# jizongFox/MI-based-Regularized-Semi-supervised-Segmentation

Hardware: NVIDIA B200
Metric: iic_mi_loss_fwd_bwd_mpixels_per_s (higher is better)
Workload: dtype f32

## Files before the change

### mi-based-regularized-semi-supervised-segmentation_b200/csrc/local_bwd_tcrb10h.cu

```cuda
#include <cuda_fp16.h>
#include <stdlib.h>

#include "common.cuh"
#include "local_kernels.cuh"
#include "tc_common.cuh"
#include "tma.cuh"

namespace iic {
namespace bwdrb10h {
using namespace tc;

constexpr int T = 3, PAD = 1;
constexpr int KP = 16;
constexpr int RMAX = 8;
constexpr int TBUF = 2 * RMAX * KP;
constexpr int APX = 272;
constexpr int MAXW = 248;
constexpr int A_CHUNK = APX * 16;
constexpr int A_SLOT = 4 * A_CHUNK;
constexpr int NA = 6;
constexpr int RAW_SLOT = 10 * 256 * 4;
constexpr int NRAW = 6;
constexpr int WROWS = T * KP;
constexpr int W_TILE = 2 * WROWS * 16;
constexpr int W_IMG = 6 * W_TILE;
constexpr int NTHREADS = 704;
constexpr int NTHREADS_FL = 704;
constexpr int SMEM_BYTES = NA * A_SLOT + 2 * W_IMG + NRAW * RAW_SLOT + 1024;
constexpr int NL = 4;
constexpr int SMEM_BYTES_FL = SMEM_BYTES + NL * RAW_SLOT;
constexpr float A_SCALE = 256.f;
constexpr int A_SCALE_LOG2 = 8;
constexpr int W_TARGET_LOG2 = 12;



#ifdef IIC_TC_TRACE
__device__ long long g_trace[4][64][6];
__device__ long long g_ctrace[32][8];
#define TRACE(role, slot) do { if (blockIdx.x == 0 && tt >= 16 && tt < 80) g_trace[role][tt - 16][slot] = clock64(); } while (0)
#define CTRACE(slot) do { if (blockIdx.x == 0 && i < 32) g_ctrace[i][slot] = clock64(); } while (0)
#else
#define TRACE(role, slot) do { } while (0)
#define CTRACE(slot) do { } while (0)
#endif

struct Params {
  int B, H, W, K;
  const float* Wc[2];
  int Kp4;
  const float* grad_loss;
  float* out[2];
  long long out_sn[2];
  int from_logits;
  float inv_temp;
  const float* lout[2];
  long long l_sn[2], l_sc[2], l_sh[2];
};

__device__ __forceinline__ uint32_t pack_h2(float a, float b) {
  const __half2 p = __floats2half2_rn(a, b);
  return *reinterpret_cast<const uint32_t*>(&p);
}
__device__ __forceinline__ uint4 pack_h8(const float* v) {
  return make_uint4(pack_h2(v[0], v[1]), pack_h2(v[2], v[3]), pack_h2(v[4], v[5]), pack_h2(v[6], v[7]));
}
__device__ __forceinline__ void split_h(float v, float& h, float& l) {
  h = __half2float(__float2half_rn(v));
  l = __half2float(__float2half_rn(v - h));
}

__device__ __forceinline__ void build_weight_row(const float* __restrict__ Wc, unsigned char* img, int e, int K, int Kp4, float wscale) {
  const int row = e % WROWS, tx = e / WROWS;
  const int ty = T - 1 - row / KP, o = row % KP;
  float w1[10], w2[10];
#pragma unroll
  for (int c = 0; c < 10; ++c) {
    const float v = (c < K && o < K) ? __ldg(Wc + ((size_t)c * T * T + ty * T + tx) * Kp4 + o) * wscale : 0.f;
    split_h(v, w1[c], w2[c]);
  }
  const float c0[8] = {w1[0], w1[1], w1[2], w1[3], w1[4], w1[5], w1[6], w1[7]};
  const float c1[8] = {w1[8], w1[9], w1[0], w1[1], w1[2], w1[3], w1[4], w1[5]};
  const float c2[8] = {w1[6], w1[7], w1[8], w1[9], w2[0], w2[1], w2[2], w2[3]};
  const float c3[8] = {w2[4], w2[5], w2[6], w2[7], w2[8], w2[9], 0.f, 0.f};
  uint4* t = reinterpret_cast<uint4*>(img + (size_t)tx * 2 * W_TILE);
  t[row] = pack_h8(c0);
  t[WROWS + row] = pack_h8(c1);
  t[2 * WROWS + row] = pack_h8(c2);
  t[3 * WROWS + row] = pack_h8(c3);
}

struct Chunk { int n, h0, nr, q0; bool cont_next; };
__device__ __forceinline__ Chunk next_chunk(long long r, long long R0, long long R1, int H, int rc) {
  Chunk c;
  c.n = (int)(r / H);
  c.h0 = (int)(r - (long long)c.n * H);
  int run = H - c.h0;
  if (run > R1 - r) run = (int)(R1 - r);
  c.nr = rc < run ? rc : run;
  if (run - c.nr == 1 && c.nr >= 3) c.nr -= 1;
  c.q0 = (r > R0 && c.h0 > 0) ? 2 : 0;
  c.cont_next = c.nr < run;
  return c;
}

template <bool FROM_LOGITS>
__global__ void __launch_bounds__(FROM_LOGITS ? NTHREADS_FL : NTHREADS, 1)
local_bwd_tcrb10h_kernel(const __grid_constant__ CUtensorMap map0, const __grid_constant__ CUtensorMap map1, const Params P) {
  extern __shared__ __align__(1024) unsigned char smem_dyn[];
  __shared__ __align__(8) uint64_t raw_full[NRAW], raw_empty[NRAW], a_full[NA], a_empty[NA], w_full, accum_full[2], tmem_ready[2];
  __shared__ __align__(8) uint64_t l_full[NL], l_empty[NL];
  __shared__ uint32_t tmem_base_s;
  __shared__ float wmax_s[4];
  __shared__ float unscale_s;
  unsigned char* smem = smem_dyn + ((1024u - (smem_u32(smem_dyn) & 1023u)) & 1023u);
  unsigned char* a_ring = smem;
  unsigned char* w_img = smem + NA * A_SLOT;
  unsigned char* raw_ring = w_img + 2 * W_IMG;
  unsigned char* l_ring = raw_ring + NRAW * RAW_SLOT;
  const int wid = threadIdx.x >> 5, lane = threadIdx.x & 31;
  const long long rows_total = (long long)P.B * P.H;
  const long long R0 = (long long)blockIdx.x * rows_total / gridDim.x;
  const long long R1 = (long long)(blockIdx.x + 1) * rows_total / gridDim.x;
  const int share = (int)(R1 - R0);
  const int nch = (share + RMAX - 1) / RMAX;
  const int rc = nch > 0 ? (share + nch - 1) / nch : RMAX;
  const int SW = P.W + 8;
  const int raw_bytes = P.K * SW * 4;
  const int ntile = P.W > 128 ? 2 : 1;

  if (threadIdx.x == 0) {
    for (int s = 0; s < NRAW; ++s) { mbar_init(&raw_full[s], 1); mbar_init(&raw_empty[s], 4); }
    for (int s = 0; s < NA; ++s) { mbar_init(&a_full[s], 4); mbar_init(&a_empty[s], 2); }
    mbar_init(&w_full, 4);
    const int ndset_i = ntile == 2 ? 2 : 1;
    for (int s = 0; s < 2; ++s) { mbar_init(&accum_full[s], 4); mbar_init(&tmem_ready[s], 4 * ndset_i); }
    for (int s = 0; s < NL; ++s) { mbar_init(&l_full[s], 1); mbar_init(&l_empty[s], 4 * ndset_i); }
    mbar_fence_init();
  }
  if (wid == 3) {
    asm volatile("tcgen05.alloc.cta_group::1.sync.aligned.shared::cta.b32 [%0], %1;" ::"r"(smem_u32(&tmem_base_s)), "r"(512));
    asm volatile("tcgen05.relinquish_alloc_permit.cta_group::1.sync.aligned;");
  }
  asm volatile("tcgen05.fence::before_thread_sync;");
  __syncthreads();
  asm volatile("tcgen05.fence::after_thread_sync;");
  const uint32_t tmem_base = tmem_base_s;

  if (wid == 0) {
    if (lane == 0) {
      tma_prefetch_desc(&map0);
      tma_prefetch_desc(&map1);
      int t = 0, s = 0;
      unsigned sph = 0;
      for (int sweep = 0; sweep < 2; ++sweep)
      for (long long r = R0; r < R1;) {
        const Chunk c = next_chunk(r, R0, R1, P.H, rc);
        for (int q = c.q0; q < c.nr + T - 1; ++q, ++t) {
          { const int tt = t; (void)tt; TRACE(0, 0); }
          if (t >= NRAW) mbar_wait(&raw_empty[s], sph ^ 1u, 1);
          { const int tt = t; (void)tt; TRACE(0, 1); }
          mbar_arrive_expect_tx(&raw_full[s], raw_bytes);
          tma_load_4d(raw_ring + s * RAW_SLOT, sweep == 0 ? &map0 : &map1, &raw_full[s], -4, c.h0 - PAD + q, 0, c.n);
          if (++s == NRAW) { s = 0; sph ^= 1u; }
        }
        r += c.nr;
      }
    }
  } else if (wid == 3) {
    if (FROM_LOGITS && lane == 0) {
      int t = 0, s = 0;
      unsigned sph = 0;
      for (int sweep = 0; sweep < 2; ++sweep)
      for (long long r = R0; r < R1;) {
        const Chunk c = next_chunk(r, R0, R1, P.H, rc);
        for (int orow = 0; orow < c.nr; ++orow, ++t) {
          if (t >= NL) mbar_wait(&l_empty[s], sph ^ 1u, 9);
          mbar_arrive_expect_tx(&l_full[s], raw_bytes);
          tma_load_4d(l_ring + s * RAW_SLOT, sweep == 0 ? &map1 : &map0, &l_full[s], -4, c.h0 + orow, 0, c.n);
          if (++s == NL) { s = 0; sph ^= 1u; }
        }
        r += c.nr;
      }
    }
  } else if (wid == 1 || wid == 2 || wid == 12 || wid == 13) {
    const int mt = (wid == 1 || wid == 12) ? 0 : 1;
    const int par = wid >= 12 ? 1 : 0;
    const bool mine = mt < ntile;
    mbar_wait(&w_full, 0u, 7);
    const uint64_t w_base0 = make_desc_kmajor_noswz(smem_u32(w_img), WROWS * 16);
    static_assert(NA % 2 == 0 && NRAW % 2 == 0, "the stage-parity split needs even ring depths");
    int a = 0, i = 0, tt = 0;
    unsigned aph = 0;
    for (int sweep = 0; sweep < 2; ++sweep)
    for (long long r = R0; r < R1; ++i) {
      const uint64_t w_base = w_base0 + (uint64_t)(sweep * (W_IMG / 16));
      const Chunk c = next_chunk(r, R0, R1, P.H, rc);
      const int buf = i & 1;
      if (lane == 0 && wid == 1) CTRACE(0);
      mbar_wait(&tmem_ready[buf], (unsigned)(i >> 1) & 1u, 6);
      if (lane == 0 && wid == 1) CTRACE(1);
      asm volatile("tcgen05.fence::after_thread_sync;");
      const int nq = c.nr + T - 1;
      const int nr_next = c.cont_next ? next_chunk(r + c.nr, R0, R1, P.H, rc).nr : 0;
      for (int q = c.q0; q < nq; ++q, ++tt) {
        if ((tt & 1) != par) {
          if (++a == NA) { a = 0; aph ^= 1u; }
          continue;
        }
        if (lane == 0 && par == 0) TRACE(1 + mt, 0);
        mbar_wait(&a_full[a], aph, 5);
        asm volatile("tcgen05.fence::after_thread_sync;");
        if (lane == 0) {
          if (par == 0) TRACE(1 + mt, 1);
          if (mine) {
            const int ty_max = q < T - 1 ? q : T - 1;
            const int ty_min = q - c.nr + 1 > 0 ? q - c.nr + 1 : 0;
            const uint32_t nn = (uint32_t)((ty_max - ty_min + 1) * KP);
            const uint32_t idesc_f16 = (1u << 4) | ((nn >> 3) << 17) | (8u << 24);
            const uint32_t d_tmem = tmem_base + (uint32_t)(buf * TBUF + (mt * RMAX + (q - ty_max)) * KP);
            const uint64_t a_12 = make_desc_kmajor_noswz(smem_u32(a_ring + a * A_SLOT), A_CHUNK) + (uint64_t)(mt * 128 + 8 - PAD);
            const uint64_t a_34 = a_12 + (uint64_t)(2 * A_CHUNK / 16);
            const uint64_t b_base = w_base + (uint64_t)((T - 1 - ty_max) * KP);
#pragma unroll
            for (int tx = 0; tx < T; ++tx) {
              const uint64_t bt = b_base + (uint64_t)tx * (2 * W_TILE / 16);
              umma_bf16(d_tmem, a_12 + (uint64_t)tx, bt, idesc_f16);
              umma_bf16(d_tmem, a_34 + (uint64_t)tx, bt + (uint64_t)(W_TILE / 16), idesc_f16);
            }
          }
        }
        if (c.cont_next && q >= c.nr) {
          mbar_wait(&tmem_ready[buf ^ 1], (unsigned)((i + 1) >> 1) & 1u, 6);
          asm volatile("tcgen05.fence::after_thread_sync;");
          if (lane == 0 && mine) {
            const int q2 = q - c.nr;
            const int ty_max = q2;
            const int ty_min = q2 - nr_next + 1 > 0 ? q2 - nr_next + 1 : 0;
            const uint32_t nn = (uint32_t)((ty_max - ty_min + 1) * KP);
            const uint32_t idesc_f16 = (1u << 4) | ((nn >> 3) << 17) | (8u << 24);
            const uint32_t d_tmem = tmem_base + (uint32_t)((buf ^ 1) * TBUF + (mt * RMAX + (q2 - ty_max)) * KP);
            const uint64_t a_12 = make_desc_kmajor_noswz(smem_u32(a_ring + a * A_SLOT), A_CHUNK) + (uint64_t)(mt * 128 + 8 - PAD);
            const uint64_t a_34 = a_12 + (uint64_t)(2 * A_CHUNK / 16);
            const uint64_t b_base = w_base + (uint64_t)((T - 1 - ty_max) * KP);
#pragma unroll
            for (int tx = 0; tx < T; ++tx) {
              const uint64_t bt = b_base + (uint64_t)tx * (2 * W_TILE / 16);
              umma_bf16(d_tmem, a_12 + (uint64_t)tx, bt, idesc_f16);
              umma_bf16(d_tmem, a_34 + (uint64_t)tx, bt + (uint64_t)(W_TILE / 16), idesc_f16);
            }
          }
        }
        if (lane == 0) {
          if (par == 0) TRACE(1 + mt, 2);
          umma_commit(&a_empty[a]);
        }
        __syncwarp();
        if (++a == NA) { a = 0; aph ^= 1u; }
      }
      if (lane == 0) umma_commit(&accum_full[buf]);
      __syncwarp();
      r += c.nr;
    }
  } else if (wid >= 4 && wid < 12) {
    const int tid = (threadIdx.x - 128) & 127;
    const int grp = wid >= 8 ? 1 : 0;
    int a = 0, s = 0, t = 0;
    unsigned aph = 0, sph = 0;
    for (int sweep = 0; sweep < 2; ++sweep)
    for (long long r = R0; r < R1;) {
      const Chunk c = next_chunk(r, R0, R1, P.H, rc);
      for (int q = c.q0; q < c.nr + T - 1; ++q, ++t) {
        if ((t & 1) != grp) {
          if (++a == NA) { a = 0; aph ^= 1u; }
          if (++s == NRAW) { s = 0; sph ^= 1u; }
          continue;
        }
        const int tt = t;
        (void)tt;
        if (tid == 0 && wid == 4) TRACE(3, 0);
        if (t >= NA) mbar_wait(&a_empty[a], aph ^ 1u, 3);
        if (tid == 0 && wid == 4) TRACE(3, 1);
        mbar_wait(&raw_full[s], sph, 4);
        if (tid == 0 && wid == 4) TRACE(3, 2);
        unsigned char* am = a_ring + a * A_SLOT;
        const float* raw = reinterpret_cast<const float*>(raw_ring + s * RAW_SLOT);
        const int srow = c.h0 - PAD + q;
        const bool row_in = srow >= 0 && srow < P.H;
        float v[2][10];
#pragma unroll
        for (int u = 0; u < 2; ++u) {
          const int px = tid + u * 128;
#pragma unroll
          for (int ch = 0; ch < 10; ++ch) v[u][ch] = (ch < P.K && px < SW) ? raw[ch * SW + px] : 0.f;
        }
#pragma unroll
        for (int u = 0; u < 2; ++u) {
          const int px = tid + u * 128;
          if (FROM_LOGITS) {
            const int col = px - 4;
            if (row_in && col >= 0 && col < P.W) {
              float mx = v[u][0];
#pragma unroll
              for (int ch = 1; ch < 10; ++ch) if (ch < P.K) mx = fmaxf(mx, v[u][ch]);
              float sum = 0.f;
#pragma unroll
              for (int ch = 0; ch < 10; ++ch) {
                v[u][ch] = ch < P.K ? __expf((v[u][ch] - mx) * P.inv_temp) : 0.f;
                sum += v[u][ch];
              }
              const float inv = 1.f / sum;
#pragma unroll
              for (int ch = 0; ch < 10; ++ch) v[u][ch] *= inv;
            } else {
#pragma unroll
              for (int ch = 0; ch < 10; ++ch) v[u][ch] = 0.f;
            }
          }
        }
        float2 hi[10], lo[10];
#pragma unroll
        for (int ch = 0; ch < 10; ++ch) {
          const float2 sv = __fmul2_rn(make_float2(v[0][ch], v[1][ch]), make_float2(A_SCALE, A_SCALE));
          hi[ch] = make_float2(__uint_as_float(__float_as_uint(sv.x) & 0xFFFFE000u), __uint_as_float(__float_as_uint(sv.y) & 0xFFFFE000u));
          lo[ch] = __ffma2_rn(hi[ch], make_float2(-1.f, -1.f), sv);
        }
#pragma unroll
        for (int u = 0; u < 2; ++u) {
          const int px = tid + u * 128;
          uint32_t hp[5], lp[5];
#pragma unroll
          for (int c2 = 0; c2 < 5; ++c2) {
            const __half2 hh = u == 0 ? __floats2half2_rn(hi[2 * c2].x, hi[2 * c2 + 1].x) : __floats2half2_rn(hi[2 * c2].y, hi[2 * c2 + 1].y);
            const __half2 ll = u == 0 ? __floats2half2_rn(lo[2 * c2].x, lo[2 * c2 + 1].x) : __floats2half2_rn(lo[2 * c2].y, lo[2 * c2 + 1].y);
            hp[c2] = *reinterpret_cast<const uint32_t*>(&hh);
            lp[c2] = *reinterpret_cast<const uint32_t*>(&ll);
          }
          if (px < SW) {
            const int off = (px + 4) * 16;
            *reinterpret_cast<uint4*>(am + off) = make_uint4(hp[0], hp[1], hp[2], hp[3]);
            *reinterpret_cast<uint4*>(am + A_CHUNK + off) = make_uint4(hp[4], lp[0], lp[1], lp[2]);
            *reinterpret_cast<uint4*>(am + 2 * A_CHUNK + off) = make_uint4(lp[3], lp[4], hp[0], hp[1]);
            *reinterpret_cast<uint4*>(am + 3 * A_CHUNK + off) = make_uint4(hp[2], hp[3], hp[4], 0u);
          }
        }
        __syncwarp();
        if (lane == 0) mbar_arrive(&raw_empty[s]);
        asm volatile("fence.proxy.async.shared::cta;" ::: "memory");
        __syncwarp();
        if (lane == 0) mbar_arrive(&a_full[a]);
        if (tid == 0 && wid == 4) TRACE(3, 3);
        if (++a == NA) { a = 0; aph ^= 1u; }
        if (++s == NRAW) { s = 0; sph ^= 1u; }
      }
      r += c.nr;
    }
  } else if (wid >= 14) {
    const int q4 = wid & 3;
    const int dset = wid >= 18 ? 1 : 0;
    const int ndset = ntile == 2 ? 2 : 1;
    const int mt0 = ndset == 2 ? dset : 0, mt1 = ndset == 2 ? dset + 1 : ntile;
    const int zc0 = ndset == 2 ? dset * RMAX * KP : 0, zc1 = ndset == 2 ? (dset + 1) * RMAX * KP : TBUF;
    float unscale = 1.f;
    const float g0 = P.grad_loss ? __ldg(P.grad_loss) : 1.f;
    const size_t plane = (size_t)P.H * P.W;
    const uint32_t lane_base = tmem_base + ((uint32_t)(q4 * 32) << 16);
    auto zero_accumulators = [&](int buf) {
      for (int c = zc0; c < zc1; c += 8)
        asm volatile("tcgen05.st.sync.aligned.32x32b.x8.b32 [%0], {%1, %1, %1, %1, %1, %1, %1, %1};" ::"r"(lane_base + buf * TBUF + c), "r"(0u) : "memory");
      asm volatile("tcgen05.wait::st.sync.aligned;" ::: "memory");
      asm volatile("tcgen05.fence::before_thread_sync;");
      __syncwarp();
      if (lane == 0) mbar_arrive(&tmem_ready[buf]);
    };
    if (dset < ndset) {
    zero_accumulators(0);
    zero_accumulators(1);
    }
    if (dset == 0) {
      const int etid = threadIdx.x - 14 * 32;
      const int ncoef = P.K * T * T * P.Kp4;
      float mx = 0.f;
      for (int e = etid; e < 2 * ncoef; e += 128) mx = fmaxf(mx, fabsf(__ldg(P.Wc[e >= ncoef] + (e >= ncoef ? e - ncoef : e))));
#pragma unroll
      for (int o = 16; o > 0; o >>= 1) mx = fmaxf(mx, __shfl_xor_sync(0xffffffffu, mx, o));
      if (lane == 0) wmax_s[q4] = mx;
      asm volatile("bar.sync 1, 128;" ::: "memory");
      mx = fmaxf(fmaxf(wmax_s[0], wmax_s[1]), fmaxf(wmax_s[2], wmax_s[3]));
      int wexp = 0;
      if (mx > 0.f && mx < 3.0e38f) wexp = W_TARGET_LOG2 - ilogbf(mx);
      if (wexp > 100) wexp = 100;
      const float wscale = scalbnf(1.f, wexp);
      unscale = scalbnf(1.f, -(wexp + A_SCALE_LOG2));
      for (int e = etid; e < 2 * 3 * WROWS; e += 128) {
        const int sweep = e / (3 * WROWS);
        build_weight_row(P.Wc[sweep], w_img + sweep * W_IMG, e - sweep * 3 * WROWS, P.K, P.Kp4, wscale);
      }
      if (etid == 0) unscale_s = unscale;
      asm volatile("fence.proxy.async.shared::cta;" ::: "memory");
      __syncwarp();
      if (lane == 0) mbar_arrive(&w_full);
    } else {
      mbar_wait(&w_full, 0u, 7);
      unscale = *reinterpret_cast<volatile float*>(&unscale_s);
    }
    const float g = g0 * unscale;
    int i = 0, ls = 0;
    unsigned lph = 0;
    for (int sweep = 0; sweep < 2 && dset < ndset; ++sweep)
    for (long long r = R0; r < R1; ++i) {
      const Chunk c = next_chunk(r, R0, R1, P.H, rc);
      const int buf = i & 1;
      if (lane == 0 && wid == 14) CTRACE(2);
      mbar_wait(&accum_full[buf], (unsigned)(i >> 1) & 1u, 8);
      if (lane == 0 && wid == 14) CTRACE(3);
      asm volatile("tcgen05.fence::after_thread_sync;");
      for (int orow = 0; orow < c.nr; orow += 2) {
        const int nrow = orow + 1 < c.nr ? 2 : 1;
        if (FROM_LOGITS) {
          mbar_wait(&l_full[ls], lph, 10);
          if (nrow == 2) mbar_wait(&l_full[(ls + 1) % NL], (ls + 1 == NL) ? (lph ^ 1u) : lph, 10);
        }
        for (int mt = mt0; mt < mt1; ++mt) {
          const int col = mt * 128 + q4 * 32 + lane;
          const bool live = col < P.W;
          uint32_t v[2][16];
#pragma unroll
          for (int h = 0; h < 2; ++h) {
            const int orh = orow + h < RMAX ? orow + h : orow;
#pragma unroll
            for (int ch = 0; ch < 16; ch += 8) {
              const uint32_t taddr = lane_base + (uint32_t)(buf * TBUF + (mt * RMAX + orh) * KP + ch);
              asm volatile("tcgen05.ld.sync.aligned.32x32b.x8.b32 {%0, %1, %2, %3, %4, %5, %6, %7}, [%8];"
                           : "=r"(v[h][ch]), "=r"(v[h][ch + 1]), "=r"(v[h][ch + 2]), "=r"(v[h][ch + 3]), "=r"(v[h][ch + 4]),
                             "=r"(v[h][ch + 5]), "=r"(v[h][ch + 6]), "=r"(v[h][ch + 7])
                           : "r"(taddr));
            }
          }
          asm volatile("tcgen05.wait::ld.sync.aligned;" ::: "memory");
          if (live) {
#pragma unroll
            for (int h = 0; h < 2; ++h) {
              if (h < nrow) {
                float* dst = P.out[sweep] + (size_t)c.n * P.out_sn[sweep] + (size_t)(c.h0 + orow + h) * P.W + col;
                if (!FROM_LOGITS) {
                  if (P.K == 10) {
#pragma unroll
                    for (int o = 0; o < 10; ++o) dst[(size_t)o * plane] = g * __uint_as_float(v[h][o]);
                  } else {
#pragma unroll
                    for (int o = 0; o < 9; ++o) dst[(size_t)o * plane] = g * __uint_as_float(v[h][o]);
                  }
                } else {
                  const float* lp = reinterpret_cast<const float*>(l_ring + ((ls + h) % NL) * RAW_SLOT) + col + 4;
                  float pr[10];
                  float mx = -3.0e38f;
#pragma unroll
                  for (int o = 0; o < 10; ++o) {
                    pr[o] = o < P.K ? lp[o * SW] : -3.0e38f;
                    mx = fmaxf(mx, pr[o]);
                  }
                  float sum = 0.f;
#pragma unroll
                  for (int o = 0; o < 10; ++o) {
                    pr[o] = o < P.K ? __expf((pr[o] - mx) * P.inv_temp) : 0.f;
                    sum += pr[o];
                  }
                  const float inv = 1.f / sum;
                  float dot = 0.f;
#pragma unroll
                  for (int o = 0; o < 10; ++o) {
                    pr[o] *= inv;
                    dot = fmaf(g * __uint_as_float(v[h][o]), pr[o], dot);
                  }
                  if (P.K == 10) {
#pragma unroll
                    for (int o = 0; o < 10; ++o) dst[(size_t)o * plane] = P.inv_temp * pr[o] * (g * __uint_as_float(v[h][o]) - dot);
                  } else {
#pragma unroll
                    for (int o = 0; o < 9; ++o) dst[(size_t)o * plane] = P.inv_temp * pr[o] * (g * __uint_as_float(v[h][o]) - dot);
                  }
                }
              }
            }
          }
        }
        if (FROM_LOGITS) {
          __syncwarp();
          for (int h = 0; h < nrow; ++h) {
            if (lane == 0) mbar_arrive(&l_empty[ls]);
            if (++ls == NL) { ls = 0; lph ^= 1u; }
          }
        }
      }
      r += c.nr;
      if (lane == 0 && wid == 14) CTRACE(4);
      zero_accumulators(buf);
      if (lane == 0 && wid == 14) CTRACE(5);
    }
  }
  asm volatile("tcgen05.fence::before_thread_sync;");
  __syncthreads();
  if (wid == 3) asm volatile("tcgen05.dealloc.cta_group::1.sync.aligned.b32 %0, %1;" ::"r"(tmem_base), "r"(512));
}

}

int local_bwd_tcrb10h_try(const LocalMaps& m, const float* Wx, const float* Wy, const LocalGrads& g, int from_logits,
                          float inv_temp, cudaStream_t st) {
  using namespace bwdrb10h;
  const int B = m.B, K = m.K, H = m.H, W = m.W, sms = m.sms;
  if ((K != 9 && K != 10) || m.pad != 1 || W % 4 != 0 || W > MAXW || W < 8) return -1;
  if ((long long)B * H < 8LL * sms && !options().tc10_force) return -1;
  CUtensorMap mx, my;
  if (!make_map_4d(&mx, m.x, m, W + 8, 1, K)) return -1;
  if (!make_map_4d(&my, m.y, m, W + 8, 1, K)) return -1;
  IIC_CHECK_RC(ensure_dyn_smem((const void*)(local_bwd_tcrb10h_kernel<false>), (int)(SMEM_BYTES)));
  IIC_CHECK_RC(ensure_dyn_smem((const void*)(local_bwd_tcrb10h_kernel<true>), (int)(SMEM_BYTES_FL)));
  const int Kp4 = (K + 3) & ~3;
  Params P{B, H, W, K, {Wx, Wy}, Kp4, g.grad_loss, {g.gx, g.gy}, {g.gx_sn, g.gy_sn}, from_logits, inv_temp, {m.x.p, m.y.p},
           {m.x.sn, m.y.sn}, {m.x.sc, m.y.sc}, {m.x.sh, m.y.sh}};
  if (from_logits) local_bwd_tcrb10h_kernel<true><<<sms, NTHREADS_FL, SMEM_BYTES_FL, st>>>(my, mx, P);
  else local_bwd_tcrb10h_kernel<false><<<sms, NTHREADS, SMEM_BYTES, st>>>(my, mx, P);
  IIC_CHECK_CUDA(cudaGetLastError());
  return 0;
}

}
```

Before: 10220.

## Fold horizontal conv taps into MMA N dimension and combine shifted outputs in epilogue

Replaces the three per-tx MMAs per row with a single wider MMA whose N dimension packs all three horizontal taps (KP 32, RMAX 4). The epilogue then sums the three tap outputs with lane shuffles, using shared-memory seam exchange across warps, and tiles columns by 126 with halo overlap. The aim is to cut the number of tensor-core instructions and weight-tile traffic per row. In exchange it adds epilogue shuffles, a named barrier per row, halved row depth per accumulator, and an extra A-ring zero-padding pass.

```diff
diff --git a/mi-based-regularized-semi-supervised-segmentation_b200/csrc/local_bwd_tcrb10h.cu b/mi-based-regularized-semi-supervised-segmentation_b200/csrc/local_bwd_tcrb10h.cu
--- a/mi-based-regularized-semi-supervised-segmentation_b200/csrc/local_bwd_tcrb10h.cu
+++ b/mi-based-regularized-semi-supervised-segmentation_b200/csrc/local_bwd_tcrb10h.cu
@@ -11,9 +11,10 @@
 using namespace tc;
 
 constexpr int T = 3, PAD = 1;
-constexpr int KP = 16;
-constexpr int RMAX = 8;
+constexpr int KP = 32;
+constexpr int RMAX = 4;
 constexpr int TBUF = 2 * RMAX * KP;
+constexpr int TILE = 126;
 constexpr int APX = 272;
 constexpr int MAXW = 248;
 constexpr int A_CHUNK = APX * 16;
@@ -23,7 +24,7 @@
 constexpr int NRAW = 6;
 constexpr int WROWS = T * KP;
 constexpr int W_TILE = 2 * WROWS * 16;
-constexpr int W_IMG = 6 * W_TILE;
+constexpr int W_IMG = 2 * W_TILE;
 constexpr int NTHREADS = 704;
 constexpr int NTHREADS_FL = 704;
 constexpr int SMEM_BYTES = NA * A_SLOT + 2 * W_IMG + NRAW * RAW_SLOT + 1024;
@@ -70,20 +71,20 @@
   l = __half2float(__float2half_rn(v - h));
 }
 
-__device__ __forceinline__ void build_weight_row(const float* __restrict__ Wc, unsigned char* img, int e, int K, int Kp4, float wscale) {
-  const int row = e % WROWS, tx = e / WROWS;
-  const int ty = T - 1 - row / KP, o = row % KP;
+__device__ __forceinline__ void build_weight_row(const float* __restrict__ Wc, unsigned char* img, int row, int K, int Kp4, float wscale) {
+  const int ty = T - 1 - row / KP, rr = row % KP;
+  const int tx = rr / 10, o = rr % 10;
   float w1[10], w2[10];
 #pragma unroll
   for (int c = 0; c < 10; ++c) {
-    const float v = (c < K && o < K) ? __ldg(Wc + ((size_t)c * T * T + ty * T + tx) * Kp4 + o) * wscale : 0.f;
+    const float v = (c < K && o < K && tx < T) ? __ldg(Wc + ((size_t)c * T * T + ty * T + tx) * Kp4 + o) * wscale : 0.f;
     split_h(v, w1[c], w2[c]);
   }
   const float c0[8] = {w1[0], w1[1], w1[2], w1[3], w1[4], w1[5], w1[6], w1[7]};
   const float c1[8] = {w1[8], w1[9], w1[0], w1[1], w1[2], w1[3], w1[4], w1[5]};
   const float c2[8] = {w1[6], w1[7], w1[8], w1[9], w2[0], w2[1], w2[2], w2[3]};
   const float c3[8] = {w2[4], w2[5], w2[6], w2[7], w2[8], w2[9], 0.f, 0.f};
-  uint4* t = reinterpret_cast<uint4*>(img + (size_t)tx * 2 * W_TILE);
+  uint4* t = reinterpret_cast<uint4*>(img);
   t[row] = pack_h8(c0);
   t[WROWS + row] = pack_h8(c1);
   t[2 * WROWS + row] = pack_h8(c2);
@@ -113,6 +114,7 @@
   __shared__ uint32_t tmem_base_s;
   __shared__ float wmax_s[4];
   __shared__ float unscale_s;
+  __shared__ float seam_s[2][2][4][2][10];
   unsigned char* smem = smem_dyn + ((1024u - (smem_u32(smem_dyn) & 1023u)) & 1023u);
   unsigned char* a_ring = smem;
   unsigned char* w_img = smem + NA * A_SLOT;
@@ -127,7 +129,7 @@
   const int rc = nch > 0 ? (share + nch - 1) / nch : RMAX;
   const int SW = P.W + 8;
   const int raw_bytes = P.K * SW * 4;
-  const int ntile = P.W > 128 ? 2 : 1;
+  const int ntile = P.W > TILE ? 2 : 1;
 
   if (threadIdx.x == 0) {
     for (int s = 0; s < NRAW; ++s) { mbar_init(&raw_full[s], 1); mbar_init(&raw_empty[s], 4); }
@@ -219,15 +221,11 @@
             const uint32_t nn = (uint32_t)((ty_max - ty_min + 1) * KP);
             const uint32_t idesc_f16 = (1u << 4) | ((nn >> 3) << 17) | (8u << 24);
             const uint32_t d_tmem = tmem_base + (uint32_t)(buf * TBUF + (mt * RMAX + (q - ty_max)) * KP);
-            const uint64_t a_12 = make_desc_kmajor_noswz(smem_u32(a_ring + a * A_SLOT), A_CHUNK) + (uint64_t)(mt * 128 + 8 - PAD);
+            const uint64_t a_12 = make_desc_kmajor_noswz(smem_u32(a_ring + a * A_SLOT), A_CHUNK) + (uint64_t)(mt * TILE + 8 - PAD);
             const uint64_t a_34 = a_12 + (uint64_t)(2 * A_CHUNK / 16);
             const uint64_t b_base = w_base + (uint64_t)((T - 1 - ty_max) * KP);
-#pragma unroll
-            for (int tx = 0; tx < T; ++tx) {
-              const uint64_t bt = b_base + (uint64_t)tx * (2 * W_TILE / 16);
-              umma_bf16(d_tmem, a_12 + (uint64_t)tx, bt, idesc_f16);
-              umma_bf16(d_tmem, a_34 + (uint64_t)tx, bt + (uint64_t)(W_TILE / 16), idesc_f16);
-            }
+            umma_bf16(d_tmem, a_12, b_base, idesc_f16);
+            umma_bf16(d_tmem, a_34, b_base + (uint64_t)(W_TILE / 16), idesc_f16);
           }
         }
         if (c.cont_next && q >= c.nr) {
@@ -240,15 +238,11 @@
             const uint32_t nn = (uint32_t)((ty_max - ty_min + 1) * KP);
             const uint32_t idesc_f16 = (1u << 4) | ((nn >> 3) << 17) | (8u << 24);
             const uint32_t d_tmem = tmem_base + (uint32_t)((buf ^ 1) * TBUF + (mt * RMAX + (q2 - ty_max)) * KP);
-            const uint64_t a_12 = make_desc_kmajor_noswz(smem_u32(a_ring + a * A_SLOT), A_CHUNK) + (uint64_t)(mt * 128 + 8 - PAD);
+            const uint64_t a_12 = make_desc_kmajor_noswz(smem_u32(a_ring + a * A_SLOT), A_CHUNK) + (uint64_t)(mt * TILE + 8 - PAD);
             const uint64_t a_34 = a_12 + (uint64_t)(2 * A_CHUNK / 16);
             const uint64_t b_base = w_base + (uint64_t)((T - 1 - ty_max) * KP);
-#pragma unroll
-            for (int tx = 0; tx < T; ++tx) {
-              const uint64_t bt = b_base + (uint64_t)tx * (2 * W_TILE / 16);
-              umma_bf16(d_tmem, a_12 + (uint64_t)tx, bt, idesc_f16);
-              umma_bf16(d_tmem, a_34 + (uint64_t)tx, bt + (uint64_t)(W_TILE / 16), idesc_f16);
-            }
+            umma_bf16(d_tmem, a_12, b_base, idesc_f16);
+            umma_bf16(d_tmem, a_34, b_base + (uint64_t)(W_TILE / 16), idesc_f16);
           }
         }
         if (lane == 0) {
@@ -265,6 +259,13 @@
   } else if (wid >= 4 && wid < 12) {
     const int tid = (threadIdx.x - 128) & 127;
     const int grp = wid >= 8 ? 1 : 0;
+    {
+      const int npx = APX - (SW + 4);
+      for (int e = tid; e < (NA / 2) * 4 * npx; e += 128) {
+        const int slot = 2 * (e / (4 * npx)) + grp, k = (e / npx) % 4, px = SW + 4 + e % npx;
+        *reinterpret_cast<uint4*>(a_ring + slot * A_SLOT + k * A_CHUNK + px * 16) = make_uint4(0u, 0u, 0u, 0u);
+      }
+    }
     int a = 0, s = 0, t = 0;
     unsigned aph = 0, sph = 0;
     for (int sweep = 0; sweep < 2; ++sweep)
@@ -359,7 +360,7 @@
     const int q4 = wid & 3;
     const int dset = wid >= 18 ? 1 : 0;
     const int ndset = ntile == 2 ? 2 : 1;
-    const int mt0 = ndset == 2 ? dset : 0, mt1 = ndset == 2 ? dset + 1 : ntile;
+    const int mt = dset;
     const int zc0 = ndset == 2 ? dset * RMAX * KP : 0, zc1 = ndset == 2 ? (dset + 1) * RMAX * KP : TBUF;
     float unscale = 1.f;
     const float g0 = P.grad_loss ? __ldg(P.grad_loss) : 1.f;
@@ -392,9 +393,9 @@
       if (wexp > 100) wexp = 100;
       const float wscale = scalbnf(1.f, wexp);
       unscale = scalbnf(1.f, -(wexp + A_SCALE_LOG2));
-      for (int e = etid; e < 2 * 3 * WROWS; e += 128) {
-        const int sweep = e / (3 * WROWS);
-        build_weight_row(P.Wc[sweep], w_img + sweep * W_IMG, e - sweep * 3 * WROWS, P.K, P.Kp4, wscale);
+      for (int e = etid; e < 2 * WROWS; e += 128) {
+        const int sweep = e / WROWS;
+        build_weight_row(P.Wc[sweep], w_img + sweep * W_IMG, e - sweep * WROWS, P.K, P.Kp4, wscale);
       }
       if (etid == 0) unscale_s = unscale;
       asm volatile("fence.proxy.async.shared::cta;" ::: "memory");
@@ -405,7 +406,7 @@
       unscale = *reinterpret_cast<volatile float*>(&unscale_s);
     }
     const float g = g0 * unscale;
-    int i = 0, ls = 0;
+    int i = 0, ls = 0, rp = 0;
     unsigned lph = 0;
     for (int sweep = 0; sweep < 2 && dset < ndset; ++sweep)
     for (long long r = R0; r < R1; ++i) {
@@ -415,82 +416,90 @@
       mbar_wait(&accum_full[buf], (unsigned)(i >> 1) & 1u, 8);
       if (lane == 0 && wid == 14) CTRACE(3);
       asm volatile("tcgen05.fence::after_thread_sync;");
-      for (int orow = 0; orow < c.nr; orow += 2) {
-        const int nrow = orow + 1 < c.nr ? 2 : 1;
-        if (FROM_LOGITS) {
-          mbar_wait(&l_full[ls], lph, 10);
-          if (nrow == 2) mbar_wait(&l_full[(ls + 1) % NL], (ls + 1 == NL) ? (lph ^ 1u) : lph, 10);
-        }
-        for (int mt = mt0; mt < mt1; ++mt) {
-          const int col = mt * 128 + q4 * 32 + lane;
-          const bool live = col < P.W;
-          uint32_t v[2][16];
-#pragma unroll
-          for (int h = 0; h < 2; ++h) {
-            const int orh = orow + h < RMAX ? orow + h : orow;
-#pragma unroll
-            for (int ch = 0; ch < 16; ch += 8) {
-              const uint32_t taddr = lane_base + (uint32_t)(buf * TBUF + (mt * RMAX + orh) * KP + ch);
-              asm volatile("tcgen05.ld.sync.aligned.32x32b.x8.b32 {%0, %1, %2, %3, %4, %5, %6, %7}, [%8];"
-                           : "=r"(v[h][ch]), "=r"(v[h][ch + 1]), "=r"(v[h][ch + 2]), "=r"(v[h][ch + 3]), "=r"(v[h][ch + 4]),
-                             "=r"(v[h][ch + 5]), "=r"(v[h][ch + 6]), "=r"(v[h][ch + 7])
-                           : "r"(taddr));
+      for (int orow = 0; orow < c.nr; ++orow, rp ^= 1) {
+        if (FROM_LOGITS) mbar_wait(&l_full[ls], lph, 10);
+        uint32_t v[30];
+        {
+          const uint32_t taddr = lane_base + (uint32_t)(buf * TBUF + (mt * RMAX + orow) * KP);
+          asm volatile("tcgen05.ld.sync.aligned.32x32b.x16.b32 {%0, %1, %2, %3, %4, %5, %6, %7, %8, %9, %10, %11, %12, %13, %14, %15}, [%16];"
+                       : "=r"(v[0]), "=r"(v[1]), "=r"(v[2]), "=r"(v[3]), "=r"(v[4]), "=r"(v[5]), "=r"(v[6]), "=r"(v[7]),
+                         "=r"(v[8]), "=r"(v[9]), "=r"(v[10]), "=r"(v[11]), "=r"(v[12]), "=r"(v[13]), "=r"(v[14]), "=r"(v[15])
+                       : "r"(taddr));
+          asm volatile("tcgen05.ld.sync.aligned.32x32b.x8.b32 {%0, %1, %2, %3, %4, %5, %6, %7}, [%8];"
+                       : "=r"(v[16]), "=r"(v[17]), "=r"(v[18]), "=r"(v[19]), "=r"(v[20]), "=r"(v[21]), "=r"(v[22]), "=r"(v[23])
+                       : "r"(taddr + 16));
+          asm volatile("tcgen05.ld.sync.aligned.32x32b.x4.b32 {%0, %1, %2, %3}, [%4];"
+                       : "=r"(v[24]), "=r"(v[25]), "=r"(v[26]), "=r"(v[27]) : "r"(taddr + 24));
+          asm volatile("tcgen05.ld.sync.aligned.32x32b.x2.b32 {%0, %1}, [%2];" : "=r"(v[28]), "=r"(v[29]) : "r"(taddr + 28));
+          asm volatile("tcgen05.wait::ld.sync.aligned;" ::: "memory");
+        }
+        float (*seam)[2][10] = seam_s[mt][rp];
+        if (lane == 31) {
+#pragma unroll
+          for (int o = 0; o < 10; ++o) seam[q4][0][o] = __uint_as_float(v[o]);
+        }
+        if (lane == 0) {
+#pragma unroll
+          for (int o = 0; o < 10; ++o) seam[q4][1][o] = __uint_as_float(v[20 + o]);
+        }
+        if (dset == 0) asm volatile("bar.sync 2, 128;" ::: "memory");
+        else asm volatile("bar.sync 3, 128;" ::: "memory");
+        float s[10];
+#pragma unroll
+        for (int o = 0; o < 10; ++o) {
+          float p0 = __shfl_up_sync(0xffffffffu, __uint_as_float(v[o]), 1);
+          float p2 = __shfl_down_sync(0xffffffffu, __uint_as_float(v[20 + o]), 1);
+          if (lane == 0) p0 = q4 > 0 ? seam[q4 - 1][0][o] : 0.f;
+          if (lane == 31) p2 = q4 < 3 ? seam[q4 + 1][1][o] : 0.f;
+          s[o] = (p0 + __uint_as_float(v[10 + o])) + p2;
+        }
+        const int tl = q4 * 32 + lane;
+        const int col = mt * TILE - 1 + tl;
+        if (tl >= 1 && tl <= TILE && col < P.W) {
+          float* dst = P.out[sweep] + (size_t)c.n * P.out_sn[sweep] + (size_t)(c.h0 + orow) * P.W + col;
+          if (!FROM_LOGITS) {
+            if (P.K == 10) {
+#pragma unroll
+              for (int o = 0; o < 10; ++o) dst[(size_t)o * plane] = g * s[o];
+            } else {
+#pragma unroll
+              for (int o = 0; o < 9; ++o) dst[(size_t)o * plane] = g * s[o];
+            }
+          } else {
+            const float* lp = reinterpret_cast<const float*>(l_ring + ls * RAW_SLOT) + col + 4;
+            float pr[10];
+            float mx = -3.0e38f;
+#pragma unroll
+            for (int o = 0; o < 10; ++o) {
+              pr[o] = o < P.K ? lp[o * SW] : -3.0e38f;
+              mx = fmaxf(mx, pr[o]);
+            }
+            float sum = 0.f;
+#pragma unroll
+            for (int o = 0; o < 10; ++o) {
+              pr[o] = o < P.K ? __expf((pr[o] - mx) * P.inv_temp) : 0.f;
+              sum += pr[o];
+            }
+            const float inv = 1.f / sum;
+            float dot = 0.f;
+#pragma unroll
+            for (int o = 0; o < 10; ++o) {
+              pr[o] *= inv;
+              dot = fmaf(g * s[o], pr[o], dot);
+            }
+            if (P.K == 10) {
+#pragma unroll
+              for (int o = 0; o < 10; ++o) dst[(size_t)o * plane] = P.inv_temp * pr[o] * (g * s[o] - dot);
+            } else {
+#pragma unroll
+              for (int o = 0; o < 9; ++o) dst[(size_t)o * plane] = P.inv_temp * pr[o] * (g * s[o] - dot);
             }
           }
-          asm volatile("tcgen05.wait::ld.sync.aligned;" ::: "memory");
-          if (live) {
-#pragma unroll
-            for (int h = 0; h < 2; ++h) {
-              if (h < nrow) {
-                float* dst = P.out[sweep] + (size_t)c.n * P.out_sn[sweep] + (size_t)(c.h0 + orow + h) * P.W + col;
-                if (!FROM_LOGITS) {
-                  if (P.K == 10) {
-#pragma unroll
-                    for (int o = 0; o < 10; ++o) dst[(size_t)o * plane] = g * __uint_as_float(v[h][o]);
-                  } else {
-#pragma unroll
-                    for (int o = 0; o < 9; ++o) dst[(size_t)o * plane] = g * __uint_as_float(v[h][o]);
-                  }
-                } else {
-                  const float* lp = reinterpret_cast<const float*>(l_ring + ((ls + h) % NL) * RAW_SLOT) + col + 4;
-                  float pr[10];
-                  float mx = -3.0e38f;
-#pragma unroll
-                  for (int o = 0; o < 10; ++o) {
-                    pr[o] = o < P.K ? lp[o * SW] : -3.0e38f;
-                    mx = fmaxf(mx, pr[o]);
-                  }
-                  float sum = 0.f;
-#pragma unroll
-                  for (int o = 0; o < 10; ++o) {
-                    pr[o] = o < P.K ? __expf((pr[o] - mx) * P.inv_temp) : 0.f;
-                    sum += pr[o];
-                  }
-                  const float inv = 1.f / sum;
-                  float dot = 0.f;
-#pragma unroll
-                  for (int o = 0; o < 10; ++o) {
-                    pr[o] *= inv;
-                    dot = fmaf(g * __uint_as_float(v[h][o]), pr[o], dot);
-                  }
-                  if (P.K == 10) {
-#pragma unroll
-                    for (int o = 0; o < 10; ++o) dst[(size_t)o * plane] = P.inv_temp * pr[o] * (g * __uint_as_float(v[h][o]) - dot);
-                  } else {
-#pragma unroll
-                    for (int o = 0; o < 9; ++o) dst[(size_t)o * plane] = P.inv_temp * pr[o] * (g * __uint_as_float(v[h][o]) - dot);
-                  }
-                }
-              }
-            }
-          }
         }
         if (FROM_LOGITS) {
           __syncwarp();
-          for (int h = 0; h < nrow; ++h) {
-            if (lane == 0) mbar_arrive(&l_empty[ls]);
-            if (++ls == NL) { ls = 0; lph ^= 1u; }
-          }
+          if (lane == 0) mbar_arrive(&l_empty[ls]);
+          if (++ls == NL) { ls = 0; lph ^= 1u; }
         }
       }
       r += c.nr;
```

Result: slower. 6240 (median of 6 runs) (-38.9%).
